# Bizilizi/stereo_reconstruction

Measured on AMD Instinct MI355X. Metric: Mdisparities/s (HxWxD / s) on Middlebury-H pairs, higher is better.
Workload: dtype u8

## Files before the change

### stereo_reconstruction_amd/csrc/ws_march_mfma.h

```cpp
#pragma once
#include "ws_march_kernel.h"

namespace wsamd {

typedef int ws_i32x4 __attribute__((ext_vector_type(4)));
typedef int ws_i32x16 __attribute__((ext_vector_type(16)));
typedef int ws_i32x2 __attribute__((ext_vector_type(2)));
typedef __attribute__((address_space(3))) ws_i32x2 lds_i64;
typedef unsigned long long ws_u64x8 __attribute__((ext_vector_type(8)));
typedef unsigned long long ws_u64x2 __attribute__((ext_vector_type(2)));

constexpr int kMfmaXWaves = 4;
constexpr int kMfmaVWaves = 2;
constexpr int kMfmaWaves = kMfmaXWaves * kMfmaVWaves;
constexpr int kMfmaVTiles = 9;
constexpr int kMfmaTilesPerWave = (kMfmaVTiles + kMfmaVWaves - 1) / kMfmaVWaves;
constexpr int kMfmaKT = 3;

constexpr int kMfmaMaxSteps = 8192;
constexpr long long kMfmaA0 = 1LL << 25, kMfmaAccPoison = 1LL << 27;
constexpr long long kMfmaG0 = 1LL << 26, kMfmaBiasPoison = 1LL << 26;
constexpr long long kMfmaC0 = 2 * kMfmaA0 + kMfmaG0;
constexpr long long kMfmaValidBound = kMfmaC0 + (1LL << 25);
template <int K, int WH>
constexpr bool mfma_key_ranges_hold()
{
    constexpr long long XB = 128LL * 128 * K * WH, EB = 128LL * K * kMfmaMaxSteps;
    static_assert(XB + EB < kMfmaA0, "Acc + A0 stays positive");
    static_assert(kMfmaA0 + XB + EB + kMfmaAccPoison < (1LL << 28), "the 4 bits shifted out of an accumulator are zeros");
    static_assert(2 * EB <= kMfmaG0, "gsum + G0 stays non-negative");
    static_assert(((kMfmaG0 + XB + 2 * EB + kMfmaBiasPoison) << kMfmaKT) + (1 << kMfmaKT) <= (1LL << 31), "a bias word is a positive int");
    static_assert(kMfmaC0 - 2 * XB >= 0, "a cost word is positive");
    static_assert(((kMfmaC0 + 3 * XB + 2 * kMfmaAccPoison + kMfmaBiasPoison) << kMfmaKT) + (1 << kMfmaKT) <= (1LL << 32),
                  "a doubly poisoned key does not wrap, and the low word of a pair does not carry");
    static_assert(kMfmaC0 + 3 * XB < kMfmaValidBound, "every valid cost word is below the bound");
    static_assert(kMfmaC0 - 2 * XB + 2 * kMfmaAccPoison >= kMfmaValidBound && kMfmaC0 - 2 * XB + kMfmaBiasPoison >= kMfmaValidBound,
                  "every poisoned cost word is at or above it");
    return true;
}

struct MfmaLds {
    int n_a, n_b;
    int rb_a, rb_b;
    int nvc;
    int o_b, o_bias, o_merge, o_op;
    int nblk;
    int bytes;
};
__host__ __device__ constexpr int mfma_ring_rows(int wh) { return wh + 4; }
__host__ __device__ constexpr int mfma_op_rows(int wh) { return wh + 2; }
__host__ __device__ inline MfmaLds mfma_lds_layout(int ww, int wh)
{
    MfmaLds l{};
    const int tx = 32 * kMfmaXWaves;
    l.nvc = tx + 32 * (kMfmaVTiles - 1);
    l.n_a = tx + 12;
    l.n_b = l.nvc + 12;
    l.rb_a = march_raw_bytes(l.n_a);
    l.rb_b = march_raw_bytes(l.n_b);
    l.o_b = mfma_ring_rows(wh) * l.rb_a;
    l.o_bias = l.o_b + mfma_ring_rows(wh) * l.rb_b;
    l.o_merge = l.o_bias + 2 * 4 * l.nvc;
    l.o_op = l.o_merge + 2 * 8 * tx;
    l.nblk = l.nvc / 32;
    l.bytes = l.o_op + mfma_op_rows(wh) * l.nblk * 1024;
    (void)ww;
    return l;
}

__device__ __forceinline__ ws_i32x4 mfma_operand(uint32_t row, uint32_t p)
{
    const lds_u32 *q = lds_at32(row + (p & ~3u));
    const uint32_t d0 = q[0], d1 = q[1], d2 = q[2], d3 = q[3], d4 = q[4];
    const uint32_t sh = p & 3u;
    ws_i32x4 r;
    r.x = (int)__builtin_amdgcn_alignbyte(d1, d0, sh);
    r.y = (int)__builtin_amdgcn_alignbyte(d2, d1, sh);
    r.z = (int)__builtin_amdgcn_alignbyte(d3, d2, sh);
    r.w = (int)__builtin_amdgcn_alignbyte(d4, d3, sh);
    return r;
}

struct MfmaRaw {
    uint32_t d0, d1, d2, d3, d4, sh;
};
__device__ __forceinline__ MfmaRaw mfma_raw_load(uint32_t t)
{
    const lds_u32 *q = lds_at32(t & ~3u);
    return MfmaRaw{q[0], q[1], q[2], q[3], q[4], t & 3u};
}
__device__ __forceinline__ ws_i32x4 mfma_raw_align(const MfmaRaw &r)
{
    ws_i32x4 v;
    v.x = (int)__builtin_amdgcn_alignbyte(r.d1, r.d0, r.sh);
    v.y = (int)__builtin_amdgcn_alignbyte(r.d2, r.d1, r.sh);
    v.z = (int)__builtin_amdgcn_alignbyte(r.d3, r.d2, r.sh);
    v.w = (int)__builtin_amdgcn_alignbyte(r.d4, r.d3, r.sh);
    return v;
}

__device__ __forceinline__ uint32_t mfma_pair_sum(uint32_t x)
{
    const auto r = __builtin_amdgcn_permlane32_swap(x, x, false, false);
    return r[0] + r[1];
}

__device__ __forceinline__ void mfma_pair_best(int &cw, int &G)
{
    const auto c = __builtin_amdgcn_permlane32_swap((uint32_t)cw, (uint32_t)cw, false, false);
    const auto q = __builtin_amdgcn_permlane32_swap((uint32_t)G, (uint32_t)G, false, false);
    const int c0 = (int)c[0], c1 = (int)c[1], g0 = (int)q[0], g1 = (int)q[1];
    const bool up = c1 < c0 || (c1 == c0 && g1 < g0);
    cw = up ? c1 : c0;
    G = up ? g1 : g0;
}

constexpr int kPipeValuA = 8;
constexpr int kPipeValu[2] = {7, 12};

struct MfmaBest {
    uint32_t k, l, t;
};
__device__ __forceinline__ uint32_t mfma_best_code(const MfmaBest &b) { return 2u * b.t + (b.k < b.l ? 1u : 0u); }
template <bool FIRST>
__device__ __forceinline__ void mfma_tile_best(const ws_i32x16 &acc, const uint4 (&b4)[4], int t, MfmaBest &best)
{
    const ws_u64x8 a = __builtin_bit_cast(ws_u64x8, acc);
    uint32_t lo[8], hi[8];
#pragma unroll
    for (int q = 0; q < 4; ++q) {
        const ws_u64x2 b = __builtin_bit_cast(ws_u64x2, b4[q]);
#pragma unroll
        for (int j = 0; j < 2; ++j) {
            const unsigned long long k = (a[2 * q + j] << (kMfmaKT + 1)) + b[j];
            lo[2 * q + j] = (uint32_t)k, hi[2 * q + j] = (uint32_t)(k >> 32);
        }
    }
    uint32_t kl = min(lo[0], lo[1]), kh = min(hi[0], hi[1]);
#pragma unroll
    for (int q = 2; q < 8; q += 2) kl = min(min(kl, lo[q]), lo[q + 1]), kh = min(min(kh, hi[q]), hi[q + 1]);
    const uint32_t km = min(kl, kh);
    if constexpr (FIRST) {
        best = MfmaBest{km, kl, (uint32_t)t};
    } else {
        const bool better = (km | ((1u << kMfmaKT) - 1u)) < best.k;
        best.k = better ? km : best.k;
        best.l = better ? kl : best.l;
        best.t = better ? (uint32_t)t : best.t;
    }
}

__device__ __forceinline__ void mfma_advance(uint32_t &at, uint32_t row, uint32_t end)
{
    at += row;
    at = at == end ? 0u : at;
}

template <int WW, int WH>
__global__ void __launch_bounds__(64 * kMfmaWaves) ws_march_mfma_kernel(const MarchArgs g)
{
    constexpr int NW = kMfmaWaves, NV = kMfmaVTiles, NVW = kMfmaTilesPerWave, KT = kMfmaKT, NT = 64 * NW, TX = 32 * kMfmaXWaves;
    constexpr int NR = mfma_ring_rows(WH);
    constexpr int K = 3 * WW;
    static_assert(K <= 32 && K > 16, "one row of the window is one K = 32 step, its pad in the upper lane half");
    static_assert(mfma_key_ranges_hold<K, WH>(), "the ranges of the packed key (above)");
    static_assert(KT == 3, "(Acc << (KT + 1)) + bias' is one v_lshl_add_u64 per register pair for a shift of 4");
    static_assert(kMfmaXWaves == 4 && kMfmaVWaves == 2, "wave >> 2 is the share of the tiles");

    extern __shared__ uint4 ws_smem4[];
    const uint32_t lds0 = (uint32_t)(uintptr_t)(lds_u32 *)reinterpret_cast<uint32_t *>(ws_smem4);
    const MfmaLds L = mfma_lds_layout(WW, WH);
    const uint32_t RBA = (uint32_t)L.rb_a, RBB = (uint32_t)L.rb_b;
    const uint32_t ringA = lds0, ringB = lds0 + (uint32_t)L.o_b, biasr = lds0 + (uint32_t)L.o_bias, mrg = lds0 + (uint32_t)L.o_merge;
    const uint32_t opB = lds0 + (uint32_t)L.o_op, OPROW = 1024u * (uint32_t)L.nblk;
    constexpr int NRO = mfma_op_rows(WH);

    const int tid = threadIdx.x, lane = tid & 63;
    const int wave = __builtin_amdgcn_readfirstlane(tid >> 6);
    const int n = lane & 31, h = lane >> 5;
    const int wx = wave & (kMfmaXWaves - 1), wv = wave >> 2;

    const int nblk = gridDim.x;
    const int logical = (blockIdx.x & 7) * (nblk >> 3) + (blockIdx.x >> 3);
    if (logical >= g.tiles * g.strips) return;
    const int tile_i = logical % g.tiles, strip_i = logical / g.tiles;
    const int tile_x0 = g.ox0 + tile_i * TX;
    const int ys = g.oy0 + strip_i * g.strip_rows;
    const int ye = min(ys + g.strip_rows, g.oy1);
    if (ys >= ye) return;

    if (g.border) {
        const bool first_t = tile_i == 0, last_t = tile_i == g.tiles - 1;
        const int cx0 = first_t ? 0 : tile_x0, cx1 = last_t ? g.out_w : tile_x0 + TX;
        auto zero_rect = [&](int x0, int x1, int y0, int y1) __attribute__((always_inline)) {
            const int w = x1 - x0, cnt = w * (y1 - y0);
            for (int i = tid; i < cnt; i += NT) {
                const int yy = y0 + i / w, xx = x0 + i % w;
                if (g.out16) g.out16[(size_t)yy * g.out_pitch + xx] = 0;
                else g.out[(size_t)yy * g.out_pitch + xx] = 0.0f;
            }
        };
        if (strip_i == 0 && g.oy0 > 0) zero_rect(cx0, cx1, 0, g.oy0);
        if (strip_i == g.strips - 1 && g.out_h > g.oy1) zero_rect(cx0, cx1, g.oy1, g.out_h);
        if (first_t && g.ox0 > 0) zero_rect(0, g.ox0, ys, ye);
        if (last_t && g.out_w > g.ox1) zero_rect(g.ox1, g.out_w, ys, ye);
    }

    for (int k = tid; k < L.o_bias / 16; k += NT) lds_store128(lds0 + 16u * (uint32_t)k, make_uint4(0u, 0u, 0u, 0u));

    const int dspan = g.d_hi - g.d_lo;
    const int vb0 = tile_x0 + g.st.boff - g.d_lo - 32 * (NV - 1);
    const int ra0 = ys + g.wy0;
    const int nsteps = (ye - ys) + WH - 1;
    const RawSide sideA = raw_side(g.st.img_a, g.st.stride_a, g.st.wa, tile_x0 + g.st.wx0, L.n_a, 0);
    const RawSide sideB = raw_side(g.st.img_b, g.st.stride_b, g.st.wb, vb0 + g.st.wx0, L.n_b, 0);
    const RawDma dmaMine = raw_dma_setup(wave == 0 ? sideA : sideB, ra0);
    const uint32_t phA0 = (uint32_t)(reinterpret_cast<uintptr_t>(sideA.base) + (uintptr_t)((long long)ra0 * sideA.stride + 3LL * sideA.c0)) & 15u;
    const uint32_t phB0 = (uint32_t)(reinterpret_cast<uintptr_t>(sideB.base) + (uintptr_t)((long long)ra0 * sideB.stride + 3LL * sideB.c0)) & 15u;
    const uint32_t stA = (uint32_t)sideA.stride & 15u, stB = (uint32_t)sideB.stride & 15u;

    const uint32_t cpBase = wave == 0 ? ringA : ringB, cpRB = wave == 0 ? RBA : RBB;
    const int ipx = -WH - g.wy0;
    uint32_t cCp, aIn, aOut, aPx, bSt, oWr, oIn, oOut, oSq, phIn, phOut, phPx, phSt;
    auto set_cursors = [&](int s) __attribute__((always_inline)) {
        auto slot = [](int i, int rows) __attribute__((always_inline)) { return (uint32_t)(((i % rows) + rows) % rows); };
        cCp = slot(s + 3, NR) * cpRB;
        aIn = slot(s, NR) * RBA, aOut = slot(s - WH, NR) * RBA, aPx = slot(s + ipx, NR) * RBA;
        bSt = slot(s + 1, NR) * RBB;
        oWr = slot(s + 1, NRO) * OPROW, oIn = slot(s, NRO) * OPROW, oOut = slot(s - WH, NRO) * OPROW, oSq = slot(s + 1 - WH, NRO) * OPROW;
        phIn = (phA0 + (uint32_t)s * stA) & 15u, phOut = (phA0 + (uint32_t)(s - WH) * stA) & 15u, phPx = (phA0 + (uint32_t)(s + ipx) * stA) & 15u;
        phSt = (phB0 + (uint32_t)(s + 1) * stB) & 15u;
    };
    auto advance = [&]() __attribute__((always_inline)) {
        mfma_advance(cCp, cpRB, (uint32_t)NR * cpRB);
        mfma_advance(aIn, RBA, (uint32_t)NR * RBA), mfma_advance(aOut, RBA, (uint32_t)NR * RBA), mfma_advance(aPx, RBA, (uint32_t)NR * RBA);
        mfma_advance(bSt, RBB, (uint32_t)NR * RBB);
        mfma_advance(oWr, OPROW, (uint32_t)NRO * OPROW), mfma_advance(oIn, OPROW, (uint32_t)NRO * OPROW);
        mfma_advance(oOut, OPROW, (uint32_t)NRO * OPROW), mfma_advance(oSq, OPROW, (uint32_t)NRO * OPROW);
        phIn = (phIn + stA) & 15u, phOut = (phOut + stA) & 15u, phPx = (phPx + stA) & 15u, phSt = (phSt + stB) & 15u;
    };

    const bool wave_on = tile_x0 + 32 * wx < g.ox1;

    ws_i32x4 amask;
#pragma unroll
    for (int j = 0; j < 4; ++j) {
        const int first = 16 * h + 4 * j;
        const int keep = K - first;
        amask[j] = keep >= 4 ? -1 : keep <= 0 ? 0 : (int)((1u << (8 * keep)) - 1u);
    }
    const uint32_t pA_lane = ringA + 3u * (uint32_t)(32 * wx + n) + 16u * (uint32_t)h;
    const uint32_t px_lane = ringA + 3u * (uint32_t)(32 * wx + n - g.st.wx0);

    __syncthreads();

    auto tiles_active = [&](int v) __attribute__((always_inline)) {
        uint32_t on = 0u;
        for (int j = 0; j < (v == 0 ? NVW : NV - NVW); ++j)
            if (32 * (NV - 1 - (v * NVW + j)) - 31 <= dspan) on |= 1u << j;
        return on;
    };

    auto march = [&](auto role, auto all) __attribute__((always_inline)) {
        constexpr int WV = decltype(role)::value;
        constexpr bool ALL = decltype(all)::value;
        constexpr int NTL = WV == 0 ? NVW : NV - NVW;
        constexpr int NI = WV == 0 ? 1 : 2;
        static_assert(kMfmaXWaves * (1 + 2) == (TX + 32 * (NV - 1)) / 32, "the waves' blocks are the tile row's");
        const uint32_t opB_lane = opB + 1024u * (uint32_t)(wx + WV * NVW) + 16u * (uint32_t)lane;

        const int blk0 = WV == 0 ? wx : kMfmaXWaves + 2 * wx;
        uint32_t gsum[NI], btag[NI];
#pragma unroll
        for (int k = 0; k < NI; ++k) {
            const int v = vb0 + 32 * (blk0 + k) + n;
            const bool bvalid = (uint32_t)(v - g.st.b_lo) <= (uint32_t)(g.st.b_hi - g.st.b_lo) && g.st.b_hi >= g.st.b_lo;
            btag[k] = (uint32_t)(((n & 3) >> 1) + 2 * (n >> 3)) + ((uint32_t)(kMfmaG0 + (bvalid ? 0 : kMfmaBiasPoison)) << KT);
            gsum[k] = 0u;
        }
        const uint32_t st_lane = ringB + 3u * (uint32_t)(32 * blk0 + n) + 16u * (uint32_t)h;
        const uint32_t it_lane = opB + 1024u * (uint32_t)blk0 + 16u * (uint32_t)lane;
        const uint32_t bi_lane = biasr + 4u * (uint32_t)(32 * blk0 + n);
        static_assert(K <= 24, "bytes 24 .. 31 of an operand entry are pad");
        const uint32_t sq_lane = opB + 1024u * (uint32_t)blk0 + 16u * (uint32_t)(32 + n) + 8u + 4u * (uint32_t)h;

        ws_i32x16 acc[NTL];
        const uint32_t active = tiles_active(WV);
#pragma unroll
        for (int j = 0; j < NTL; ++j) {
            const int t = WV * NVW + j;
#pragma unroll
            for (int i = 0; i < 16; ++i) {
                const int m = (i & 3) + 8 * (i >> 2) + 4 * h;
                const int e = 32 * (NV - 1 - t) + n - m;
                acc[j][i] = (int)((uint32_t)e <= (uint32_t)dspan ? kMfmaA0 : kMfmaA0 + kMfmaAccPoison);
            }
        }

        MfmaRaw ir[NI];
        uint32_t il[NI];
        auto items_load = [&](auto leaves) __attribute__((always_inline)) {
#pragma unroll
            for (int k = 0; k < NI; ++k) {
                ir[k] = mfma_raw_load(st_lane + 96u * (uint32_t)k + bSt + phSt);
                if constexpr (decltype(leaves)::value) il[k] = *lds_at32(sq_lane + 1024u * (uint32_t)k + oSq);
            }
        };
        MfmaRaw n_rae{}, n_ral{};
        uint4 n_bl[NTL];
        auto ahead_load = [&]() __attribute__((always_inline)) {
            n_rae = mfma_raw_load(pA_lane + aIn + phIn);
            n_ral = mfma_raw_load(pA_lane + aOut + phOut);
#pragma unroll
            for (int t = 0; t < NTL; ++t) n_bl[t] = lds_load128(opB_lane + oOut + 1024u * (uint32_t)t);
            items_load(std::true_type());
        };
        uint32_t iu_[NI];
        auto items_enter = [&](int k) __attribute__((always_inline)) {
            ws_i32x4 c = mfma_raw_align(ir[k]);
            c ^= (int)0x80808080u;
            lds_store128(it_lane + 1024u * (uint32_t)k + oWr, make_uint4((uint32_t)c.x, (uint32_t)c.y, (uint32_t)c.z, (uint32_t)c.w));
            const ws_i32x4 cm = c & amask;
            int q = 0, t = 0;
#pragma unroll
            for (int j = 0; j < 4; ++j) {
                q = __builtin_amdgcn_sdot4(c[j], cm[j], q, false);
                t = __builtin_amdgcn_sdot4(cm[j], 0x01010101, t, false);
            }
            *reinterpret_cast<lds_u32 *>((uintptr_t)(sq_lane + 1024u * (uint32_t)k + oWr)) = (uint32_t)q;
            iu_[k] = (uint32_t)q + 2u * (uint32_t)t;
        };
        auto items_leave = [&](int iu, int k, auto leaves) __attribute__((always_inline)) {
            uint32_t u = iu_[k];
            if constexpr (decltype(leaves)::value) u -= il[k];
            gsum[k] += mfma_pair_sum(u);
            *reinterpret_cast<lds_u32 *>((uintptr_t)(bi_lane + 4u * (uint32_t)((iu & 1) * L.nvc + 32 * k))) = (gsum[k] << KT) + btag[k];
        };
        auto items_finish = [&](int iu, auto leaves) __attribute__((always_inline)) {
#pragma unroll
            for (int k = 0; k < NI; ++k) {
                items_enter(k);
                items_leave(iu, k, leaves);
            }
        };

        int my_cw = 0, my_G = 0;
        struct Flush {
            ws_i32x2 o;
            uint32_t q0, q1, sh;
        };
        auto flush_load = [&](int sp) __attribute__((always_inline)) {
            Flush f;
            f.o = *reinterpret_cast<const lds_i64 *>((uintptr_t)(mrg + 8u * (uint32_t)((sp & 1) * TX + 32 * wx + n)));
            const uint32_t p = px_lane + aPx + phPx;
            const lds_u32 *q = lds_at32(p & ~3u);
            f.q0 = q[0], f.q1 = q[1], f.sh = p & 3u;
            return f;
        };
        auto flush_store = [&](int sp, const Flush &f) __attribute__((always_inline)) {
            int cw = my_cw, G = my_G;
            if (f.o.x < cw || (f.o.x == cw && f.o.y < G)) { cw = f.o.x; G = f.o.y; }
            const int x = tile_x0 + 32 * wx + n, y = ys + sp - (WH - 1);
            if (h == 0 && x < g.ox1) {
                float val;
                if (cw >= (int)kMfmaValidBound) val = g.fallback_neg ? -(float)x : (float)x;
                else val = (float)(g.d_lo + 32 * (NV - 1) + n - G);
                if ((__builtin_amdgcn_alignbyte(f.q1, f.q0, f.sh) & 0x00ffffffu) == 0u) val = 0.0f;
                if (g.out16) g.out16[(size_t)y * g.out_pitch + x] = (int16_t)(int)val;
                else g.out[(size_t)y * g.out_pitch + x] = val;
            }
        };

        auto step = [&](int s, auto phase) __attribute__((always_inline)) {
            constexpr int PHASE = decltype(phase)::value;
            constexpr bool STEADY = PHASE == 2;
            constexpr bool PIPE = ALL && PHASE >= 2;
            using Leaves = std::integral_constant<bool, (PHASE >= 1)>;
            Flush fl{};
            if constexpr (WV == 1 && PHASE >= 2) {
                if (wave_on) fl = flush_load(s - 1);
            }
            if constexpr (WV == 0) {
                if (wave < 2 && (STEADY || s + 3 < nsteps)) raw_dma(cpBase + cCp, dmaMine, s + 3, lane);
            }
            const bool stage = STEADY || (s + 1 >= 0 && s + 1 < nsteps);
            if constexpr (STEADY) {
                if (!(PIPE && wave_on)) items_load(Leaves());
            }
            if (PHASE >= 0 && wave_on) {
                MfmaRaw rae{}, ral{};
                if constexpr (PIPE) {
                    rae = n_rae, ral = n_ral;
                } else {
                    rae = mfma_raw_load(pA_lane + aIn + phIn);
                    if constexpr (PHASE >= 2) ral = mfma_raw_load(pA_lane + aOut + phOut);
                }
                const uint32_t opBe = opB_lane + oIn, opBl = opB_lane + oOut;
                (void)opBl;
                if constexpr (!PIPE) {
                    if constexpr (STEADY) items_finish(s + 1, Leaves());
                    else if (stage) { items_load(Leaves()); items_finish(s + 1, Leaves()); }
                }
                ws_i32x4 ae{}, al{};
                if constexpr (!PIPE) {
                    ae = (mfma_raw_align(rae) ^ (int)0x7f7f7f7fu) & amask;
                    if constexpr (PHASE >= 2) al = (mfma_raw_align(ral) ^ (int)0x80808080u) & amask;
                }
                MfmaBest best{UINT_MAX, UINT_MAX, 0u};
                const uint32_t brow = biasr + 4u * (uint32_t)((s & 1) * L.nvc + 32 * (wx + WV * NVW) + 4 * h);
                if constexpr (PIPE) {
                    uint4 be4[NTL], bq[2][4];
#pragma unroll
                    for (int t = 0; t < NTL; ++t) be4[t] = lds_load128(opBe + 1024u * (uint32_t)t);
#pragma unroll
                    for (int q = 0; q < 4; ++q) bq[0][q] = lds_load128(brow + 4u * (uint32_t)(8 * q));
                    __builtin_amdgcn_sched_barrier(0);
                    auto enter = [&](int t) __attribute__((always_inline)) {
                        const ws_i32x4 be = {(int)be4[t].x, (int)be4[t].y, (int)be4[t].z, (int)be4[t].w};
                        acc[t] = __builtin_amdgcn_mfma_i32_32x32x32_i8(be, ae, acc[t], 0, 0, 0);
                    };
                    auto leave = [&](int t) __attribute__((always_inline)) {
                        const ws_i32x4 bl = {(int)n_bl[t].x, (int)n_bl[t].y, (int)n_bl[t].z, (int)n_bl[t].w};
                        acc[t] = __builtin_amdgcn_mfma_i32_32x32x32_i8(bl, al, acc[t], 0, 0, 0);
                    };
                    constexpr int VG = kPipeValu[WV];
                    ae = (mfma_raw_align(rae) ^ (int)0x7f7f7f7fu) & amask;
                    al = (mfma_raw_align(ral) ^ (int)0x80808080u) & amask;
#pragma unroll
                    for (int t = 0; t < NTL - 2; ++t) enter(t);
                    if constexpr (STEADY) items_enter(0);
                    __builtin_amdgcn_sched_group_barrier(0x2, kPipeValuA, 0);
#pragma unroll
                    for (int t = 0; t < NTL - 2; ++t) {
                        __builtin_amdgcn_sched_group_barrier(0x8, 1, 0);
                        __builtin_amdgcn_sched_group_barrier(0x2, VG, 0);
                    }
                    __builtin_amdgcn_sched_barrier(0);
                    enter(NTL - 2), enter(NTL - 1);
                    if constexpr (STEADY) {
                        if constexpr (NI == 2) items_enter(1);
                        else items_leave(s + 1, 0, Leaves());
                    }
                    __builtin_amdgcn_sched_group_barrier(0x8, 1, 0);
                    __builtin_amdgcn_sched_group_barrier(0x2, VG, 0);
                    __builtin_amdgcn_sched_group_barrier(0x8, 1, 0);
                    __builtin_amdgcn_sched_group_barrier(0x2, VG, 0);
                    __builtin_amdgcn_sched_barrier(0);
                    if constexpr (!STEADY) {
                        if (stage) { items_load(Leaves()); items_finish(s + 1, Leaves()); }
                    }
                    leave(0), leave(1);
                    if constexpr (STEADY && NI == 2) items_leave(s + 1, 0, Leaves());
                    __builtin_amdgcn_sched_group_barrier(0x8, 1, 0);
                    __builtin_amdgcn_sched_group_barrier(0x2, VG, 0);
                    __builtin_amdgcn_sched_group_barrier(0x8, 1, 0);
                    __builtin_amdgcn_sched_group_barrier(0x2, VG, 0);
                    __builtin_amdgcn_sched_barrier(0);
                    if constexpr (STEADY && NI == 2) {
                        items_leave(s + 1, 1, Leaves());
                        __builtin_amdgcn_sched_barrier(0);
                    }
                    advance();
#pragma unroll
                    for (int t = 0; t < NTL; ++t) {
                        if (t == NTL - 2) ahead_load();
                        if (t + 1 < NTL) {
#pragma unroll
                            for (int q = 0; q < 4; ++q) bq[(t + 1) & 1][q] = lds_load128(brow + 4u * (uint32_t)(32 * (t + 1) + 8 * q));
                        }
                        __builtin_amdgcn_sched_barrier(0);
                        if (t + 2 < NTL) {
                            leave(t + 2);
                            __builtin_amdgcn_sched_group_barrier(0x8, 1, 0);
                        }
                        if (t == 0) mfma_tile_best<true>(acc[t], bq[t & 1], t, best);
                        else mfma_tile_best<false>(acc[t], bq[t & 1], t, best);
                    }
                } else
#pragma unroll
                for (int t = 0; t < NTL; ++t) {
                    if constexpr (!ALL) {
                        if (!(active & (1u << t))) continue;
                    }
                    const uint4 be4 = lds_load128(opBe + 1024u * (uint32_t)t);
                    const ws_i32x4 be = {(int)be4.x, (int)be4.y, (int)be4.z, (int)be4.w};
                    acc[t] = __builtin_amdgcn_mfma_i32_32x32x32_i8(be, ae, acc[t], 0, 0, 0);
                    if constexpr (PHASE >= 2) {
                        const uint4 bl4 = lds_load128(opBl + 1024u * (uint32_t)t);
                        const ws_i32x4 bl = {(int)bl4.x, (int)bl4.y, (int)bl4.z, (int)bl4.w};
                        acc[t] = __builtin_amdgcn_mfma_i32_32x32x32_i8(bl, al, acc[t], 0, 0, 0);
                    }
                    if constexpr (PHASE >= 1) {
                        uint4 b4[4];
#pragma unroll
                        for (int q = 0; q < 4; ++q) b4[q] = lds_load128(brow + 4u * (uint32_t)(32 * t + 8 * q));
                        if (ALL && t == 0) mfma_tile_best<true>(acc[t], b4, t, best);
                        else mfma_tile_best<false>(acc[t], b4, t, best);
                    }
                }
                if constexpr (PHASE >= 1) {
                    const uint32_t bestc = mfma_best_code(best);
                    const int i_best = 2 * (int)(best.k & ((1u << KT) - 1u)) + (int)(bestc & 1u);
                    int G = 32 * ((int)(bestc >> 1) + WV * NVW) + (i_best & 3) + 8 * (i_best >> 2) + 4 * h;
                    int cw = (int)(best.k >> KT);
                    mfma_pair_best(cw, G);
                    if constexpr (WV == 1 && PHASE >= 2) flush_store(s - 1, fl);
                    if constexpr (WV == 0) {
                        *reinterpret_cast<lds_i64 *>((uintptr_t)(mrg + 8u * (uint32_t)((s & 1) * TX + 32 * wx + n))) = ws_i32x2{cw, G};
                    } else {
                        my_cw = cw;
                        my_G = G;
                    }
                }
            } else {
                if constexpr (STEADY) items_finish(s + 1, Leaves());
                else if (stage) { items_load(Leaves()); items_finish(s + 1, Leaves()); }
            }
            if constexpr (WV == 0) {
                if (wave < 2) dma_wait();
            }
            __syncthreads();
            if constexpr (PIPE) {
                if (!wave_on) advance();
            } else {
                advance();
                if constexpr (ALL && PHASE == 1) {
                    if (wave_on) ahead_load();
                }
            }
        };

        int s = -3;
        set_cursors(s);
#pragma unroll 1
        for (; s < 0; ++s) step(s, std::integral_constant<int, -1>());
#pragma unroll 1
        for (; s < WH - 1; ++s) step(s, std::integral_constant<int, 0>());
        step(s++, std::integral_constant<int, 1>());
#pragma unroll 1
        for (; s + 3 < nsteps; ++s) step(s, std::integral_constant<int, 2>());
#pragma unroll 1
        for (; s < nsteps; ++s) step(s, std::integral_constant<int, 3>());
        if constexpr (WV == 1) {
            if (wave_on) flush_store(nsteps - 1, flush_load(nsteps - 1));
        }
    };
    const bool all = tiles_active(wv) == (1u << (wv == 0 ? NVW : NV - NVW)) - 1u;
    if (wv == 0) {
        if (all) march(std::integral_constant<int, 0>(), std::true_type());
        else march(std::integral_constant<int, 0>(), std::false_type());
    } else {
        if (all) march(std::integral_constant<int, 1>(), std::true_type());
        else march(std::integral_constant<int, 1>(), std::false_type());
    }
}

}
```

Before: 5.612 million.

## Compute window square and plain sums by per-centre DPP box filter instead of per-item dots

```diff
diff --git a/stereo_reconstruction_amd/csrc/ws_march_mfma.h b/stereo_reconstruction_amd/csrc/ws_march_mfma.h
--- a/stereo_reconstruction_amd/csrc/ws_march_mfma.h
+++ b/stereo_reconstruction_amd/csrc/ws_march_mfma.h
@@ -99,12 +99,6 @@
     return v;
 }
 
-__device__ __forceinline__ uint32_t mfma_pair_sum(uint32_t x)
-{
-    const auto r = __builtin_amdgcn_permlane32_swap(x, x, false, false);
-    return r[0] + r[1];
-}
-
 __device__ __forceinline__ void mfma_pair_best(int &cw, int &G)
 {
     const auto c = __builtin_amdgcn_permlane32_swap((uint32_t)cw, (uint32_t)cw, false, false);
@@ -116,7 +110,7 @@
 }
 
 constexpr int kPipeValuA = 8;
-constexpr int kPipeValu[2] = {7, 12};
+constexpr int kPipeValu[2] = {6, 6};
 
 struct MfmaBest {
     uint32_t k, l, t;
@@ -270,19 +264,28 @@
         const uint32_t opB_lane = opB + 1024u * (uint32_t)(wx + WV * NVW) + 16u * (uint32_t)lane;
 
         const int blk0 = WV == 0 ? wx : kMfmaXWaves + 2 * wx;
-        uint32_t gsum[NI], btag[NI];
-#pragma unroll
-        for (int k = 0; k < NI; ++k) {
-            const int v = vb0 + 32 * (blk0 + k) + n;
-            const bool bvalid = (uint32_t)(v - g.st.b_lo) <= (uint32_t)(g.st.b_hi - g.st.b_lo) && g.st.b_hi >= g.st.b_lo;
-            btag[k] = (uint32_t)(((n & 3) >> 1) + 2 * (n >> 3)) + ((uint32_t)(kMfmaG0 + (bvalid ? 0 : kMfmaBiasPoison)) << KT);
-            gsum[k] = 0u;
-        }
         const uint32_t st_lane = ringB + 3u * (uint32_t)(32 * blk0 + n) + 16u * (uint32_t)h;
         const uint32_t it_lane = opB + 1024u * (uint32_t)blk0 + 16u * (uint32_t)lane;
-        const uint32_t bi_lane = biasr + 4u * (uint32_t)(32 * blk0 + n);
+        const uint32_t it_hi = it_lane + (h == 0 ? 8u : 0u);
+        constexpr int CW = 64 - (WW - 1), NVC = TX + 32 * (NV - 1), kSumShift = 13;
+        static_assert(WW * 3 * 128 * 128 < (1 << (32 - kSumShift)) && WW * 3 * 255 < (1 << kSumShift), "both window sums fit their fields of the packed word");
+        static_assert((NVC + CW - 1) / CW <= NW && NVC >= CW, "a chunk per wave covers the tile row's centres");
+        const int chunk = WV * kMfmaXWaves + wx;
+        const int cp0 = min(CW * chunk, NVC - CW);
+        const int cv = min(cp0 + lane, NVC - 1);
+        const bool c_own = lane < CW;
+        uint32_t gsum = 0u, btag;
+        {
+            const int v = vb0 + cv, nn = cv & 31;
+            const bool bvalid = (uint32_t)(v - g.st.b_lo) <= (uint32_t)(g.st.b_hi - g.st.b_lo) && g.st.b_hi >= g.st.b_lo;
+            btag = (uint32_t)(((nn & 3) >> 1) + 2 * (nn >> 3)) + ((uint32_t)(kMfmaG0 + (bvalid ? 0 : kMfmaBiasPoison)) << KT);
+        }
+        const uint32_t cs_lane = ringB + 3u * (uint32_t)(cp0 + lane);
         static_assert(K <= 24, "bytes 24 .. 31 of an operand entry are pad");
-        const uint32_t sq_lane = opB + 1024u * (uint32_t)blk0 + 16u * (uint32_t)(32 + n) + 8u + 4u * (uint32_t)h;
+        const uint32_t pad_lane = opB + 1024u * (uint32_t)(cv >> 5) + 16u * (uint32_t)(32 + (cv & 31)) + 8u;
+        const uint32_t sq_lane = pad_lane + (c_own ? 0u : 4u);
+        const uint32_t bi_lane = c_own ? biasr + 4u * (uint32_t)cv : pad_lane + 4u;
+        const uint32_t bi_par = c_own ? 4u * (uint32_t)L.nvc : 0u;
 
         ws_i32x16 acc[NTL];
         const uint32_t active = tiles_active(WV);
@@ -298,13 +301,15 @@
         }
 
         MfmaRaw ir[NI];
-        uint32_t il[NI];
+        uint32_t cd0 = 0u, cd1 = 0u, csh = 0u;
+        uint32_t il = 0u;
         auto items_load = [&](auto leaves) __attribute__((always_inline)) {
 #pragma unroll
-            for (int k = 0; k < NI; ++k) {
-                ir[k] = mfma_raw_load(st_lane + 96u * (uint32_t)k + bSt + phSt);
-                if constexpr (decltype(leaves)::value) il[k] = *lds_at32(sq_lane + 1024u * (uint32_t)k + oSq);
-            }
+            for (int k = 0; k < NI; ++k) ir[k] = mfma_raw_load(st_lane + 96u * (uint32_t)k + bSt + phSt);
+            const uint32_t at = cs_lane + bSt + phSt;
+            const lds_u32 *q = lds_at32(at & ~3u);
+            cd0 = q[0], cd1 = q[1], csh = at & 3u;
+            if constexpr (decltype(leaves)::value) il = *lds_at32(sq_lane + oSq);
         };
         MfmaRaw n_rae{}, n_ral{};
         uint4 n_bl[NTL];
@@ -315,33 +320,36 @@
             for (int t = 0; t < NTL; ++t) n_bl[t] = lds_load128(opB_lane + oOut + 1024u * (uint32_t)t);
             items_load(std::true_type());
         };
-        uint32_t iu_[NI];
         auto items_enter = [&](int k) __attribute__((always_inline)) {
-            ws_i32x4 c = mfma_raw_align(ir[k]);
-            c ^= (int)0x80808080u;
-            lds_store128(it_lane + 1024u * (uint32_t)k + oWr, make_uint4((uint32_t)c.x, (uint32_t)c.y, (uint32_t)c.z, (uint32_t)c.w));
-            const ws_i32x4 cm = c & amask;
-            int q = 0, t = 0;
-#pragma unroll
-            for (int j = 0; j < 4; ++j) {
-                q = __builtin_amdgcn_sdot4(c[j], cm[j], q, false);
-                t = __builtin_amdgcn_sdot4(cm[j], 0x01010101, t, false);
-            }
-            *reinterpret_cast<lds_u32 *>((uintptr_t)(sq_lane + 1024u * (uint32_t)k + oWr)) = (uint32_t)q;
-            iu_[k] = (uint32_t)q + 2u * (uint32_t)t;
-        };
-        auto items_leave = [&](int iu, int k, auto leaves) __attribute__((always_inline)) {
-            uint32_t u = iu_[k];
-            if constexpr (decltype(leaves)::value) u -= il[k];
-            gsum[k] += mfma_pair_sum(u);
-            *reinterpret_cast<lds_u32 *>((uintptr_t)(bi_lane + 4u * (uint32_t)((iu & 1) * L.nvc + 32 * k))) = (gsum[k] << KT) + btag[k];
+            const ws_i32x4 cm = (mfma_raw_align(ir[k]) ^ (int)0x80808080u) & amask;
+            *reinterpret_cast<lds_i64 *>((uintptr_t)(it_hi + 1024u * (uint32_t)k + oWr)) = ws_i32x2{cm.z, cm.w};
+            *reinterpret_cast<lds_i64 *>((uintptr_t)(it_lane + 1024u * (uint32_t)k + oWr)) = ws_i32x2{cm.x, cm.y};
+        };
+        uint32_t cbox = 0u;
+        auto sums_box = [&]() __attribute__((always_inline)) {
+            const uint32_t x = __builtin_amdgcn_alignbyte(cd1, cd0, csh);
+            const int c = (int)((x ^ 0x80808080u) & 0x00ffffffu);
+            const uint32_t q = (uint32_t)__builtin_amdgcn_sdot4(c, c, 0, false);
+            const uint32_t r = __builtin_amdgcn_udot4(x, 0x00010101u, 0u, false);
+            const uint32_t w = (q << kSumShift) + r;
+            uint32_t s = w;
+#pragma unroll
+            for (int j = 1; j < WW; ++j) s = w + (uint32_t)__builtin_amdgcn_mov_dpp((int)s, 0x130, 0xf, 0xf, true);
+            cbox = s;
+        };
+        auto sums_leave = [&](int iu, auto leaves) __attribute__((always_inline)) {
+            const uint32_t q = cbox >> kSumShift, r = cbox & ((1u << kSumShift) - 1u);
+            uint32_t u = q + 2u * r - 2u * 128u * (uint32_t)K;
+            if constexpr (decltype(leaves)::value) u -= il;
+            gsum += u;
+            *reinterpret_cast<lds_u32 *>((uintptr_t)(sq_lane + oWr)) = q;
+            *reinterpret_cast<lds_u32 *>((uintptr_t)(bi_lane + (uint32_t)(iu & 1) * bi_par)) = (gsum << KT) + btag;
         };
         auto items_finish = [&](int iu, auto leaves) __attribute__((always_inline)) {
 #pragma unroll
-            for (int k = 0; k < NI; ++k) {
-                items_enter(k);
-                items_leave(iu, k, leaves);
-            }
+            for (int k = 0; k < NI; ++k) items_enter(k);
+            sums_box();
+            sums_leave(iu, leaves);
         };
 
         int my_cw = 0, my_G = 0;
@@ -439,7 +447,7 @@
                     enter(NTL - 2), enter(NTL - 1);
                     if constexpr (STEADY) {
                         if constexpr (NI == 2) items_enter(1);
-                        else items_leave(s + 1, 0, Leaves());
+                        else sums_box();
                     }
                     __builtin_amdgcn_sched_group_barrier(0x8, 1, 0);
                     __builtin_amdgcn_sched_group_barrier(0x2, VG, 0);
@@ -450,14 +458,17 @@
                         if (stage) { items_load(Leaves()); items_finish(s + 1, Leaves()); }
                     }
                     leave(0), leave(1);
-                    if constexpr (STEADY && NI == 2) items_leave(s + 1, 0, Leaves());
+                    if constexpr (STEADY) {
+                        if constexpr (NI == 2) sums_box();
+                        else sums_leave(s + 1, Leaves());
+                    }
                     __builtin_amdgcn_sched_group_barrier(0x8, 1, 0);
                     __builtin_amdgcn_sched_group_barrier(0x2, VG, 0);
                     __builtin_amdgcn_sched_group_barrier(0x8, 1, 0);
                     __builtin_amdgcn_sched_group_barrier(0x2, VG, 0);
                     __builtin_amdgcn_sched_barrier(0);
                     if constexpr (STEADY && NI == 2) {
-                        items_leave(s + 1, 1, Leaves());
+                        sums_leave(s + 1, Leaves());
                         __builtin_amdgcn_sched_barrier(0);
                     }
                     advance();
```

New measurement: 5.831 million (median of 6 runs). +3.9%, better.
